# ec-jrc/lisflood-code

Hardware: AMD Instinct MI355X
Metric: Mcell-steps/s kinematic routing (higher is better)
Workload: dtype f64

## Files before the change

### lisflood-code_amd/csrc/lf_soil.hip

```cpp
#include <algorithm>
#include <cmath>
#include <cstdlib>

#include "lf_common.h"
#include "lf_canopy.h"
#include "lf_math.h"
#include "lf_soil_math.h"

namespace {

constexpr double kMaxSoilSubSteps = 1048576.0;

constexpr int kBlock = 256;
constexpr int kMaxVeg = 16;

__global__ void __launch_bounds__(kBlock) k_interception(lf_interception_args A)
{
    const long long pix = (long long)blockIdx.x * kBlock + threadIdx.x;
    if (pix >= A.N) return;
    const double rain = A.Rain[pix];
    for (long long veg = 0; veg < A.V; ++veg) {
        const long long i = veg * A.N + pix;
        const double lai = A.LAI[i];
        double smax;
        if (lai <= .1)
            smax = 0.;
        else if (lai <= 43.3)
            smax = 0.935 + 0.498 * lai - 0.00575 * (lai * lai);
        else
            smax = 11.718;
        double cum = A.CumInterception[i], inter;
        if (smax > 0) {
            double v = smax - cum;
            v = dmin(v, smax * (1. - exp(-0.046 * lai * rain / smax)));
            v = dmin(v, rain);
            inter = v;
            cum += inter;
        } else
            inter = 0.;
        double ta, drain;
        if (cum > 0.) {
            ta = dmax(dmin(cum, A.TaInterceptionMax[i]), 0.);
            cum = dmax(cum - ta, 0.);
            drain = A.drainageK * cum;
            cum = dmax(cum - drain, 0.);
        } else {
            ta = 0.;
            drain = 0.;
        }
        A.Interception[i] = inter;
        A.TaInterception[i] = ta;
        A.LeafDrainage[i] = drain;
        A.CumInterception[i] = cum;
    }
}

struct veg_plan {
    int mode[kMaxVeg];
    int landuse[kMaxVeg];
    int drained[kMaxVeg];
    int paddy_row[kMaxVeg];
};

constexpr int kClasses = 128;
constexpr int kLoopFields = 7 * 3 + 1;
constexpr int kColsPerWave = 20;
constexpr int kTile = 256;
#ifndef LF_STRAG_CAP
#define LF_STRAG_CAP 48
#endif
constexpr int kStragCap = LF_STRAG_CAP;
constexpr int kStragFields = 40;
#ifndef LF_STRAG_GROUP
#define LF_STRAG_GROUP 16
#endif
constexpr int kStragGroup = LF_STRAG_GROUP;

__device__ __forceinline__ double row_prev(double x)
{
    const int lo = __builtin_amdgcn_update_dpp(0, __double2loint(x), 0x111, 0xf, 0xf, true);
    const int hi = __builtin_amdgcn_update_dpp(0, __double2hiint(x), 0x111, 0xf, 0xf, true);
    return __hiloint2double(hi, lo);
}
__device__ __forceinline__ double row_next(double x)
{
    const int lo = __builtin_amdgcn_update_dpp(0, __double2loint(x), 0x101, 0xf, 0xf, true);
    const int hi = __builtin_amdgcn_update_dpp(0, __double2hiint(x), 0x101, 0xf, 0xf, true);
    return __hiloint2double(hi, lo);
}

template <bool FASTPOW>
__device__ __forceinline__ double layer_loop(unsigned int layer, double w, double wres, double ws, double ks, double im,
                                             double m, double k, bool pore, long long nsub, long long trips, double DtDay)
{
    const double dtsub = DtDay / (double)nsub;
    double av = w - wres, wt = w, cap = ws - w, sum = 0.;
#if LF_SOIL_HOISTED_RCP
    const soil_den D = soil_den_of(ws, wres);
#endif
    for (long long s = 0; s < trips; ++s) {
#if LF_SOIL_HOISTED_RCP
        if (s > 0) k = unsat_k_r<FASTPOW>(wt, pore, wres, D, ks, im, m);
#else
        if (s > 0) k = unsat_k<FASTPOW>(wt, pore, wres, ws, ks, im, m);
#endif
        const double cap_below = row_next(cap);
        const double limit = (layer == 2u) ? av : cap_below;
        const double flux = dmin(k * dtsub, limit);
        const double flux_above = row_prev(flux);
        const double net = (layer == 0u) ? -flux : flux_above - flux;
        const bool live = s < nsub;
        av = live ? av + net : av;
        wt = av + wres;
        cap = ws - wt;
        sum = live ? sum + flux : sum;
    }
    return sum;
}

struct soil_tail {
    double w1a, w1b, w2, inf, pref, uz, uzout, gwp, ws1a;
    double sd1a, sd1b, sd2, wwp1a, wwp1b, wwp1, wwp2, wfc1a, wfc1b, wfc1, wfc2;
    int flags;
};

__device__ __forceinline__ void soil_finish(const lf_soil_args &A, long long i, bool drained, const soil_tail &T, double sa,
                                            double sb, double sg)
{
    const bool frozen = (T.flags & 1) != 0, pore1a = (T.flags & 2) != 0, pore1b = (T.flags & 4) != 0, pore2 = (T.flags & 8) != 0;
    if (frozen) sa = sb = sg = 0.;
    double w1a = T.w1a - sa;
    const double w1b = T.w1b + sa - sb;
    const double w2 = T.w2 + sb - sg;
    const double w1 = w1a + w1b;
    const double inf = T.inf - dmax(w1a - T.ws1a, 0.);
    w1a = dmin(w1a, T.ws1a);
    double uz = T.uz, uzout = T.uzout;
    if (drained) {
        uzout += A.DrainedFraction * sg;
        uz += (1 - A.DrainedFraction) * sg + T.pref;
    } else
        uz += sg + T.pref;
    const double perc = dmin(T.gwp, uz);
    uz = dmax(uz - perc, 0.);
    A.SeepTopToSubA[i] = sa;
    A.SeepTopToSubB[i] = sb;
    A.SeepSubToGW[i] = sg;
    A.Infiltration[i] = inf;
    A.W1a[i] = w1a;
    A.W1b[i] = w1b;
    A.W1[i] = w1;
    A.W2[i] = w2;
    if (A.Theta1a) A.Theta1a[i] = pore1a ? w1a / T.sd1a : 0.;
    if (A.Theta1b) A.Theta1b[i] = pore1b ? w1b / T.sd1b : 0.;
    if (A.Theta2) A.Theta2[i] = pore2 ? w2 / T.sd2 : 0.;
    if (A.Sat1a) A.Sat1a[i] = (w1a - T.wwp1a) / (T.wfc1a - T.wwp1a);
    if (A.Sat1b) A.Sat1b[i] = (w1b - T.wwp1b) / (T.wfc1b - T.wwp1b);
    if (A.Sat1) A.Sat1[i] = (w1 - T.wwp1) / (T.wfc1 - T.wwp1);
    if (A.Sat2) A.Sat2[i] = (w2 - T.wwp2) / (T.wfc2 - T.wwp2);
    A.UZOutflow[i] = uzout;
    A.GwPercUZLZ[i] = perc;
    A.UZ[i] = uz;
}

struct soil_strag {
    double *rec;
    unsigned short *key;
    unsigned int *count;
    int trip_cap;
};

template <bool FASTPOW, bool DERIVED, bool CANOPY>
__global__ void __launch_bounds__(kTile) __attribute__((amdgpu_waves_per_eu(3)))
k_soil_fused(lf_soil_args A, veg_plan P, unsigned short *__restrict__ all_list, unsigned int *__restrict__ all_count,
             soil_strag G, unsigned int tile0, unsigned int tiles_per_veg, lf_canopy_args C, const double *__restrict__ ESRef)
{
    constexpr int kLoopCap = kTile / 2;
    __shared__ unsigned int s_count, s_next, s_all, s_strag;
    __shared__ double s_rec[kLoopFields * kLoopCap];
    __shared__ double s_res[3 * kLoopCap];
    __shared__ unsigned int s_key[kLoopCap];
    __shared__ unsigned short s_order[kLoopCap];
    __shared__ double s_stage[kStragFields * kStragCap];
    if (threadIdx.x == 0) {
        s_count = 0;
        s_next = 0;
        s_all = 0;
        s_strag = 0;
    }
    __syncthreads();
    const long long N = A.N;
    const double DtDay = A.DtDay;
    const unsigned int tile = tile0 + blockIdx.x;
    const int veg = (int)(tile / tiles_per_veg);
    const long long pix = (long long)(tile - (unsigned int)veg * tiles_per_veg) * kTile + threadIdx.x;
    const int mode = P.mode[veg];
    bool active = pix < N && mode != 0;
    if (active && mode == 2 && !A.paddy_inactive[(long long)P.paddy_row[veg] * N + pix]) active = false;
    const long long i = (long long)veg * N + pix, j = (long long)P.landuse[veg] * N + pix;

    soil_tail T;
    T.w1a = T.w1b = T.w2 = T.inf = T.pref = T.uz = T.uzout = T.gwp = T.ws1a = 0.;
    T.sd1a = T.sd1b = T.sd2 = 1.;
    T.wwp1a = T.wwp1b = T.wwp1 = T.wwp2 = 0.;
    T.wfc1a = T.wfc1b = T.wfc1 = T.wfc2 = 1.;
    T.flags = 0;
    double sa = 0, sb = 0, sg = 0;
    double k1a = 0, k1b = 0, k2 = 0, nsub_f = 1;
    unsigned int rank = 0xffffffffu;
    if (active) {
        const double in_rain = A.Rain[pix], in_snow = A.SnowMelt[pix];
        double in_leaf, in_int, in_w1a, in_w1b, in_w1, in_esmax;
        lf_canopy::column_in cin = {};
        double c_ewref = 0., c_etref = 0., c_esref = 0.;
        unsigned char c_frozen = 0;
        if (CANOPY) {
            cin = lf_canopy::load(C, veg, i, j);
            c_ewref = C.EWRef[pix];
            c_etref = C.ETRef[pix];
            c_esref = ESRef[pix];
            c_frozen = A.isFrozenSoil[pix];
        } else {
            in_leaf = A.LeafDrainage[i]; in_int = A.Interception[i];
            in_w1a = A.W1a[i]; in_w1b = A.W1b[i]; in_w1 = A.W1[i];
            in_esmax = A.ESMax[i];
        }
        const double in_dslr = A.DSLR[i], in_w2 = A.W2[i];
        const double in_uz = A.UZ[i];
        const double in_store = A.StoreMaxPervious[j];
        const double in_bx = A.b_Xinanjiang[pix], in_pinf = A.PowerInfPot[pix], in_ppref = A.PowerPrefFlow[pix];
        const double in_uzk = A.UpperZoneK[pix];
        T.gwp = A.GwPercStep[pix];
        T.sd1a = A.SoilDepth1a[j]; T.sd1b = A.SoilDepth1b[j]; T.sd2 = A.SoilDepth2[j];
        T.wwp1a = A.WWP1a[j]; T.wwp1b = A.WWP1b[j]; T.wwp2 = A.WWP2[j];
        T.wfc1a = A.WFC1a[j]; T.wfc1b = A.WFC1b[j]; T.wfc2 = A.WFC2[j];
        const double ks1a = A.KSat1a[j], ks1b = A.KSat1b[j], ks2 = A.KSat2[j];
        const double m1a = A.GenuM1a[j], m1b = A.GenuM1b[j], m2 = A.GenuM2[j];
        const double wres1a = A.WRes1a[j], wres1b = A.WRes1b[j], wres2 = A.WRes2[j];
        const double ws1a = A.WS1a[j], ws1b = A.WS1b[j], ws2 = A.WS2[j];
        T.ws1a = ws1a;
        if (CANOPY) {
            const lf_canopy::column_out o = lf_canopy::compute(C, veg, pix, i, j, cin, in_rain, c_ewref, c_etref, c_frozen != 0);
            in_leaf = o.leaf_drainage; in_int = o.interception;
            in_w1a = o.w1a; in_w1b = o.w1b; in_w1 = o.w1;
            in_esmax = c_esref * cin.lai_term;
        }
        const bool is_frozen = A.isFrozenSoil[pix] != 0;
        double im1a, im1b, im2, in_wres1, in_ws1;
        int flags;
        if (DERIVED) {
            im1a = 1 / m1a; im1b = 1 / m1b; im2 = 1 / m2;
            in_ws1 = ws1a + ws1b; in_wres1 = wres1a + wres1b;
            T.wfc1 = T.wfc1a + T.wfc1b; T.wwp1 = T.wwp1a + T.wwp1b;
            flags = (is_frozen ? 1 : 0) | ((T.sd1a != 0 && ws1a != 0) ? 2 : 0) | ((T.sd1b != 0 && ws1b != 0) ? 4 : 0) |
                    ((T.sd2 != 0 && ws2 != 0) ? 8 : 0);
        } else {
            im1a = A.GenuInvM1a[j]; im1b = A.GenuInvM1b[j]; im2 = A.GenuInvM2[j];
            in_ws1 = A.WS1[j]; in_wres1 = A.WRes1[j];
            T.wfc1 = A.WFC1[j]; T.wwp1 = A.WWP1[j];
            flags = (is_frozen ? 1 : 0) | (A.PoreSpaceNotZero1a[j] != 0 ? 2 : 0) | (A.PoreSpaceNotZero1b[j] != 0 ? 4 : 0) |
                    (A.PoreSpaceNotZero2[j] != 0 ? 8 : 0);
        }
        T.flags = flags;
        const bool frozen = (flags & 1) != 0, pore1a = (flags & 2) != 0, pore1b = (flags & 4) != 0, pore2 = (flags & 8) != 0;
        double awi = dmax((in_rain + in_snow) + in_leaf - in_int, 0.);
        double dslr = in_dslr;
        if (awi > A.AvWaterThreshold)
            dslr = 1;
        else
            dslr += DtDay;
        double esact, w1a = in_w1a, w1b = in_w1b;
        if (frozen)
            esact = 0.;
        else {
            esact = in_esmax * (sqrt(dslr) - sqrt(dslr - 1));
            esact = dmax(dmin(esact, in_w1 - in_wres1), 0.);
            const double supply1a = w1a - wres1a;
            const double es1a = dmin(esact, supply1a);
            const double es1b = dmax(esact - supply1a, 0.);
            w1a = dmax(w1a - es1a, wres1a);
            w1b = dmax(w1b - es1b, wres1b);
        }
        const double w1_ = w1a + w1b;
        const double relsat1 = pore1a ? dmin(w1_ / in_ws1, 1.0) : 0.0;
        const double satfrac = 1.0 - powxy<FASTPOW>(1.0 - relsat1, in_bx);
        const double infpot = frozen ? 0.0 : in_store * powxy<FASTPOW>(1. - satfrac, in_pinf) * DtDay;
        const double pref = powxy<FASTPOW>(relsat1, in_ppref) * awi;
        awi -= pref;
        const double inf = dmax(dmin(awi, infpot), 0.);
        const double test1a = w1a + inf;
        w1a = dmin(ws1a, test1a);
        w1b += dmax(test1a - ws1a, 0.);
        const double w2 = in_w2;
        T.w1a = w1a; T.w1b = w1b; T.w2 = w2; T.inf = inf; T.pref = pref;
        A.DSLR[i] = dslr;
        A.ESAct[i] = esact;
        A.PrefFlow[i] = pref;
        A.AvailableWaterForInfiltration[i] = awi;
        T.uzout = dmin(in_uzk * in_uz, in_uz);
        T.uz = dmax(in_uz - T.uzout, 0.);
        {
            const double w_[3] = {w1a, w1b, w2}, wres_[3] = {wres1a, wres1b, wres2}, ws_[3] = {ws1a, ws1b, ws2};
            const double ks_[3] = {ks1a, ks1b, ks2}, im_[3] = {im1a, im1b, im2}, m_[3] = {m1a, m1b, m2};
            const bool pore_[3] = {pore1a, pore1b, pore2};
            double k_[3];
            unsat_k3<FASTPOW>(w_, pore_, wres_, ws_, ks_, im_, m_, k_);
            k1a = k_[0], k1b = k_[1], k2 = k_[2];
        }
        const double av1a = w1a - wres1a, av1b = w1b - wres1b, av2 = w2 - wres2;
        const double ca = (av1a == 0) ? 0. : k1a * DtDay / av1a;
        const double cb = (av1b == 0) ? 0. : k1b * DtDay / av1b;
        const double cg = (av2 == 0) ? 0. : k2 * DtDay / av2;
        const double courant = dmax(dmax(ca, cb), cg);
        nsub_f = dmin(dmax(1., ceil(courant / A.CourantCrit)), kMaxSoilSubSteps);
#ifdef LF_SOIL_DEBUG_MAXTRIPS
        nsub_f = dmin(nsub_f, (double)LF_SOIL_DEBUG_MAXTRIPS);
#endif
        if (frozen) nsub_f = 1.;
        if (nsub_f > 1.) {
            long long c = (long long)nsub_f;
            c = c < kClasses - 1 ? c : kClasses - 1;
            const unsigned short key = (unsigned short)(threadIdx.x | ((int)c << 8));
            all_list[(size_t)tile * kTile + atomicAdd(&s_all, 1u)] = key;
            unsigned int sr = 0xffffffffu;
            if (G.trip_cap > 0 && nsub_f > (double)G.trip_cap) sr = atomicAdd(&s_strag, 1u);
            if (sr < (unsigned int)kStragCap) {
                double *R = s_stage + sr * kStragFields;
                R[0] = w1a; R[1] = wres1a; R[2] = ws1a; R[3] = ks1a; R[4] = im1a; R[5] = m1a; R[6] = k1a;
                R[7] = w1b; R[8] = wres1b; R[9] = ws1b; R[10] = ks1b; R[11] = im1b; R[12] = m1b; R[13] = k1b;
                R[14] = w2; R[15] = wres2; R[16] = ws2; R[17] = ks2; R[18] = im2; R[19] = m2; R[20] = k2;
                R[21] = (double)flags; R[22] = nsub_f; R[23] = (double)threadIdx.x;
                R[24] = inf; R[25] = pref; R[26] = T.uz; R[27] = T.uzout; R[28] = T.gwp;
                R[29] = T.sd1a; R[30] = T.sd1b; R[31] = T.sd2;
                R[32] = T.wwp1a; R[33] = T.wwp1b; R[34] = T.wwp1; R[35] = T.wwp2;
                R[36] = T.wfc1a; R[37] = T.wfc1b; R[38] = T.wfc1; R[39] = T.wfc2;
                G.key[(size_t)tile * kStragCap + sr] = key;
            } else {
                rank = atomicAdd(&s_count, 1u);
                if (rank < (unsigned int)kLoopCap) {
#define REC(f, v) s_rec[(f) * kLoopCap + rank] = (v)
                    REC(0, w1a); REC(1, wres1a); REC(2, ws1a); REC(3, ks1a); REC(4, im1a); REC(5, m1a); REC(6, k1a);
                    REC(7, w1b); REC(8, wres1b); REC(9, ws1b); REC(10, ks1b); REC(11, im1b); REC(12, m1b); REC(13, k1b);
                    REC(14, w2); REC(15, wres2); REC(16, ws2); REC(17, ks2); REC(18, im2); REC(19, m2); REC(20, k2);
                    REC(21, (double)flags);
#undef REC
                    s_key[rank] = (unsigned int)nsub_f;
                }
            }
        } else {
            sa = dmin(k1a * DtDay, ws1b - w1b);
            sb = dmin(k1b * DtDay, ws2 - w2);
            sg = dmin(k2 * DtDay, av2);
        }
    }
    __syncthreads();
    const unsigned int count = (unsigned int)__builtin_amdgcn_readfirstlane((int)s_count);
    {
        const unsigned int ns = s_strag < (unsigned int)kStragCap ? s_strag : (unsigned int)kStragCap;
        if (threadIdx.x == 0) {
            all_count[tile] = s_all;
            if (G.trip_cap > 0) G.count[tile] = ns;
        }
        double *dst = G.rec + (size_t)tile * kStragCap * kStragFields;
        for (unsigned int idx = threadIdx.x; idx < ns * kStragFields; idx += kTile) dst[idx] = s_stage[idx];
    }
    for (unsigned int base = 0; base < count; base += kLoopCap) {
        if (base > 0) {
            __syncthreads();
            if (threadIdx.x == 0) s_next = 0;
            const unsigned int r = rank - base;
            if (r < (unsigned int)kLoopCap) {
#define REC(f, v) s_rec[(f) * kLoopCap + r] = (v)
                REC(0, T.w1a); REC(1, A.WRes1a[j]); REC(2, T.ws1a); REC(3, A.KSat1a[j]); REC(4, DERIVED ? 1 / A.GenuM1a[j] : A.GenuInvM1a[j]); REC(5, A.GenuM1a[j]); REC(6, k1a);
                REC(7, T.w1b); REC(8, A.WRes1b[j]); REC(9, A.WS1b[j]); REC(10, A.KSat1b[j]); REC(11, DERIVED ? 1 / A.GenuM1b[j] : A.GenuInvM1b[j]); REC(12, A.GenuM1b[j]); REC(13, k1b);
                REC(14, T.w2); REC(15, A.WRes2[j]); REC(16, A.WS2[j]); REC(17, A.KSat2[j]); REC(18, DERIVED ? 1 / A.GenuM2[j] : A.GenuInvM2[j]); REC(19, A.GenuM2[j]); REC(20, k2);
                REC(21, (double)T.flags);
#undef REC
                s_key[r] = (unsigned int)nsub_f;
            }
            __syncthreads();
        }
        const unsigned int n = (count - base) < (unsigned int)kLoopCap ? (count - base) : (unsigned int)kLoopCap;
        if (threadIdx.x < n) {
            const unsigned int k = s_key[threadIdx.x];
            unsigned int pos = 0;
            for (unsigned int q = 0; q < n; ++q) {
                const unsigned int kq = s_key[q];
                pos += (kq > k || (kq == k && q < threadIdx.x)) ? 1u : 0u;
            }
            s_order[pos] = (unsigned short)threadIdx.x;
        }
        __syncthreads();
        const unsigned int ntasks = (n + kColsPerWave - 1) / kColsPerWave, lane = threadIdx.x & 63u;
        const unsigned int in_row = lane & 15u, col_in_row = in_row / 3u, layer = in_row - 3u * col_in_row;
        const unsigned int col = (lane >> 4) * 5u + col_in_row;
        for (;;) {
            unsigned int t = 0;
            if (lane == 0) t = atomicAdd(&s_next, 1u);
            t = (unsigned int)__builtin_amdgcn_readfirstlane((int)t);
            if (t >= ntasks) break;
            const unsigned int e = t * kColsPerWave + col;
            const bool valid = col_in_row < 5u && e < n;
            const unsigned int first = s_order[t * kColsPerWave];
            const unsigned int slot = valid ? s_order[e] : first;
            const double *__restrict__ R = s_rec + (7u * layer) * kLoopCap + slot;
            const double w = R[0], wres = R[kLoopCap], ws = R[2 * kLoopCap], ks = R[3 * kLoopCap], im = R[4 * kLoopCap],
                         m = R[5 * kLoopCap], k0 = R[6 * kLoopCap];
            const int fl = (int)s_rec[21 * kLoopCap + slot];
            const bool pore = ((fl >> (1 + (int)layer)) & 1) != 0;
            const long long trips = (long long)__builtin_amdgcn_readfirstlane((int)s_key[first]);
            const long long nsub = (long long)s_key[slot];
            const double sum = layer_loop<FASTPOW>(layer, w, wres, ws, ks, im, m, k0, pore, valid ? nsub : 0, trips, DtDay);
            if (valid) s_res[layer * kLoopCap + slot] = sum;
        }
        __syncthreads();
        const unsigned int r = rank - base;
        if (r < (unsigned int)kLoopCap) {
            sa = s_res[r];
            sb = s_res[kLoopCap + r];
            sg = s_res[2 * kLoopCap + r];
        }
    }
    if (!active) return;
    soil_finish(A, i, P.drained[veg] != 0, T, sa, sb, sg);
}

template <bool FASTPOW>
__global__ void __launch_bounds__(kTile) k_soil_stragglers(lf_soil_args A, veg_plan P, soil_strag G, unsigned int group0,
                                                           unsigned int ntiles, unsigned int tiles_per_veg)
{
    constexpr int kMaxEntries = kStragGroup * kStragCap;
    static_assert(kClasses <= kTile && kClasses % 64 == 0 && kStragCap < 256 && kStragGroup < 256, "list layout");
    __shared__ unsigned int off[kStragGroup + 1], h[kClasses], base[kClasses], next_task;
    __shared__ unsigned short cls_of[kMaxEntries], rank_of[kMaxEntries], ent_of[kMaxEntries];
    __shared__ unsigned short entry[kMaxEntries];
    const unsigned int t0 = (group0 + blockIdx.x) * kStragGroup;
    if (threadIdx.x < kClasses) h[threadIdx.x] = 0;
    if (threadIdx.x == 0) {
        unsigned int t = 0;
        for (int g = 0; g < kStragGroup; ++g) {
            off[g] = t;
            t += (t0 + g < ntiles) ? G.count[t0 + g] : 0;
        }
        off[kStragGroup] = t;
        next_task = 0;
    }
    __syncthreads();
    const unsigned int total = off[kStragGroup];
    if (total == 0) return;
    for (unsigned int q = threadIdx.x; q < total; q += kTile) {
        unsigned int g = 0;
        while (off[g + 1] <= q) ++g;
        const unsigned int sl = q - off[g];
        const unsigned int cls = G.key[(size_t)(t0 + g) * kStragCap + sl] >> 8;
        cls_of[q] = (unsigned short)cls;
        ent_of[q] = (unsigned short)((g << 8) | sl);
        rank_of[q] = (unsigned short)atomicAdd(&h[cls], 1u);
    }
    __syncthreads();
    if (threadIdx.x < 64) {
        constexpr int per = kClasses / 64;
        unsigned int mine_sum = 0;
#pragma unroll
        for (int q = 0; q < per; ++q) mine_sum += h[threadIdx.x * per + q];
        unsigned int incl = mine_sum;
#pragma unroll
        for (int d = 1; d < 64; d <<= 1) {
            const unsigned int up = __shfl_up(incl, d, 64);
            if ((int)threadIdx.x >= d) incl += up;
        }
        unsigned int acc = incl - mine_sum;
#pragma unroll
        for (int q = 0; q < per; ++q) {
            base[threadIdx.x * per + q] = acc;
            acc += h[threadIdx.x * per + q];
        }
    }
    __syncthreads();
    for (unsigned int q = threadIdx.x; q < total; q += kTile) entry[base[cls_of[q]] + rank_of[q]] = ent_of[q];
    __syncthreads();
    const unsigned int ntasks = (total + kColsPerWave - 1) / kColsPerWave, lane = threadIdx.x & 63u;
    const unsigned int in_row = lane & 15u, col_in_row = in_row / 3u, layer = in_row - 3u * col_in_row;
    const unsigned int col = (lane >> 4) * 5u + col_in_row;
    for (;;) {
        unsigned int t = 0;
        if (lane == 0) t = atomicAdd(&next_task, 1u);
        t = (unsigned int)__builtin_amdgcn_readfirstlane((int)t);
        if (t >= ntasks) break;
        const unsigned int e = t * kColsPerWave + col;
        const bool valid = col_in_row < 5u && e < total;
        const unsigned int ent = entry[total - 1u - (valid ? e : t * kColsPerWave)];
        const unsigned int tile = t0 + (ent >> 8);
        const double *__restrict__ R = G.rec + ((size_t)tile * kStragCap + (ent & 0xffu)) * kStragFields;
        const double *__restrict__ L = R + 7u * layer;
        const double w = L[0], wres = L[1], ws = L[2], ks = L[3], im = L[4], m = L[5], k0 = L[6];
        const int fl = (int)R[21];
        const bool pore = ((fl >> (1 + (int)layer)) & 1) != 0;
        const int nsub = valid ? (int)R[22] : 0;
        int trips = nsub;
#pragma unroll
        for (int d = 32; d >= 1; d >>= 1) {
            const int o = __shfl_xor(trips, d, 64);
            trips = o > trips ? o : trips;
        }
        const double sum = layer_loop<FASTPOW>(layer, w, wres, ws, ks, im, m, k0, pore, nsub, trips, A.DtDay);
        const double sb = row_next(sum);
        const double sg = row_next(sb);
        if (valid && layer == 0u) {
            soil_tail T;
            T.w1a = R[0]; T.w1b = R[7]; T.w2 = R[14]; T.ws1a = R[2]; T.flags = fl;
            T.inf = R[24]; T.pref = R[25]; T.uz = R[26]; T.uzout = R[27]; T.gwp = R[28];
            T.sd1a = R[29]; T.sd1b = R[30]; T.sd2 = R[31];
            T.wwp1a = R[32]; T.wwp1b = R[33]; T.wwp1 = R[34]; T.wwp2 = R[35];
            T.wfc1a = R[36]; T.wfc1b = R[37]; T.wfc1 = R[38]; T.wfc2 = R[39];
            const int veg = (int)(tile / tiles_per_veg);
            const long long pix = (long long)(tile - (unsigned int)veg * tiles_per_veg) * kTile + (long long)R[23];
            soil_finish(A, (long long)veg * A.N + pix, P.drained[veg] != 0, T, sum, sb, sg);
        }
    }
}

int make_plan(const lf_soil_args *a, const uint8_t *paddy_any, veg_plan *P)
{
    if (a->V > kMaxVeg) return lf_set_error(LF_E_INVALID, "V = %lld exceeds the supported maximum %d", (long long)a->V, kMaxVeg);
    int count_paddy = 0;
    for (int veg = 0; veg < (int)a->V; ++veg) {
        P->landuse[veg] = (int)a->index_landuse_all[veg];
        if (P->landuse[veg] < 0 || P->landuse[veg] >= a->L)
            return lf_set_error(LF_E_INVALID, "index_landuse_all[%d] = %d out of range", veg, P->landuse[veg]);
        P->paddy_row[veg] = 0;
        if (a->is_paddy_irrig && a->is_paddy_irrig[veg]) {
            if (!paddy_any || !paddy_any[count_paddy]) {
                P->mode[veg] = 0;
                P->drained[veg] = 0;
                continue;
            }
            P->mode[veg] = 2;
            P->drained[veg] = 0;
            P->paddy_row[veg] = count_paddy++;
        } else {
            P->mode[veg] = 1;
            P->drained[veg] = (a->is_irrigated && a->is_irrigated[veg] && a->DrainedFraction > 0) ? 1 : 0;
        }
    }
    return LF_OK;
}

inline int blocks_for(int64_t n) { return (int)((n + kBlock - 1) / kBlock); }
constexpr int kSoilTripCap = 6;

}

extern "C" {

int lf_interception_device(int device, const lf_interception_args *a)
{
    if (!a) return lf_set_error(LF_E_INVALID, "null argument");
    lf_device_ctx *c;
    LF_TRY(lf_ctx(device, &c));
    if (a->N > 0 && a->V > 0)
        hipLaunchKernelGGL(k_interception, dim3(blocks_for(a->N)), dim3(kBlock), 0, c->stream, *a);
    LF_HIP(hipGetLastError());
    return LF_OK;
}

struct soil_ws_layout {
    size_t all_count, all_list, s_count, s_key, s_rec, bytes;
};
static soil_ws_layout soil_layout(size_t ntiles)
{
    auto up = [](size_t x) { return (x + 255) & ~(size_t)255; };
    soil_ws_layout L;
    L.all_count = 0;
    L.all_list = up(sizeof(unsigned int) * (ntiles + 4));
    L.s_count = L.all_list + up(sizeof(unsigned short) * ntiles * kTile);
    L.s_key = L.s_count + up(sizeof(unsigned int) * (ntiles + 4));
    L.s_rec = L.s_key + up(sizeof(unsigned short) * ntiles * kStragCap);
    L.bytes = L.s_rec + sizeof(double) * ntiles * kStragCap * kStragFields;
    return L;
}

int lf_soil_last_deferred(int device, int64_t *count)
{
    if (!count) return lf_set_error(LF_E_INVALID, "null argument");
    lf_device_ctx *c;
    LF_TRY(lf_ctx(device, &c));
    *count = 0;
    if (!c->soil_ws || c->soil_ntiles == 0) return LF_OK;
    std::vector<unsigned int> h(c->soil_ntiles);
    LF_HIP(hipMemcpyAsync(h.data(), c->soil_ws, sizeof(unsigned int) * c->soil_ntiles, hipMemcpyDeviceToHost, c->stream));
    LF_HIP(hipStreamSynchronize(c->stream));
    int64_t tot = 0;
    for (unsigned int v : h) tot += v;
    *count = tot;
    return LF_OK;
}

int lf_soil_substep_histogram(int device, int64_t *hist, int nbins)
{
    if (!hist || nbins < 2) return lf_set_error(LF_E_INVALID, "null argument");
    lf_device_ctx *c;
    LF_TRY(lf_ctx(device, &c));
    for (int k = 0; k < nbins; ++k) hist[k] = 0;
    if (!c->soil_ws || c->soil_ntiles == 0) return LF_OK;
    const size_t nt = c->soil_ntiles;
    const soil_ws_layout L = soil_layout(nt);
    std::vector<unsigned int> cnt(nt);
    std::vector<unsigned short> lst(nt * kTile);
    LF_HIP(hipMemcpyAsync(cnt.data(), (const char *)c->soil_ws + L.all_count, sizeof(unsigned int) * nt, hipMemcpyDeviceToHost, c->stream));
    LF_HIP(hipMemcpyAsync(lst.data(), (const char *)c->soil_ws + L.all_list, sizeof(unsigned short) * nt * kTile,
                          hipMemcpyDeviceToHost, c->stream));
    LF_HIP(hipStreamSynchronize(c->stream));
    for (size_t t = 0; t < nt; ++t)
        for (unsigned int k = 0; k < cnt[t] && k < (unsigned int)kTile; ++k) {
            const int cls = lst[t * kTile + k] >> 8;
            hist[cls < nbins - 1 ? cls : nbins - 1] += 1;
        }
    return LF_OK;
}

static int soil_columns_device(int device, const lf_soil_args *a, bool derived, const lf_canopy_args *canopy = nullptr,
                               const double *esref = nullptr);

int lf_soil_columns_device(int device, const lf_soil_args *a) { return soil_columns_device(device, a, false); }

int lf_soil_columns_device_derived(int device, const lf_soil_args *a) { return soil_columns_device(device, a, true); }

int lf_land_columns_device(int device, const lf_canopy_args *canopy, const lf_soil_args *soil, const double *ESRef_dev, int derived)
{
    if (!canopy || !soil || !ESRef_dev || !canopy->index_landuse || !soil->index_landuse_all)
        return lf_set_error(LF_E_INVALID, "null argument");
    if (canopy->V != soil->V || canopy->N != soil->N || canopy->L != soil->L || soil->V != soil->L)
        return lf_set_error(LF_E_INVALID, "land columns: canopy and soil must have the same V = L and N");
    for (int v = 0; v < (int)soil->V; ++v)
        if (canopy->index_landuse[v] != v || soil->index_landuse_all[v] != v || (soil->is_paddy_irrig && soil->is_paddy_irrig[v]))
            return lf_set_error(LF_E_INVALID, "land columns: needs index_landuse[v] == v and no paddy fraction (use the "
                                "separate entry points otherwise)");
    if ((canopy->WFilla || canopy->WFillb) && (!canopy->WFilla || !canopy->WFillb || !canopy->WPF3a || !canopy->WPF3b))
        return lf_set_error(LF_E_INVALID, "wateruse: WFilla, WFillb, WPF3a and WPF3b are needed together");
    const bool same = canopy->W1a == soil->W1a && canopy->W1b == soil->W1b && canopy->W1 == soil->W1 &&
                      canopy->Interception == soil->Interception && canopy->LeafDrainage == soil->LeafDrainage &&
                      canopy->Rain == soil->Rain && canopy->isFrozenSoil == soil->isFrozenSoil &&
                      canopy->WWP1a == soil->WWP1a && canopy->WWP1b == soil->WWP1b && canopy->WFC1a == soil->WFC1a &&
                      canopy->WFC1b == soil->WFC1b;
    if (!same) return lf_set_error(LF_E_INVALID, "land columns: canopy and soil arguments name different vectors");
    return soil_columns_device(device, soil, derived != 0, canopy, ESRef_dev);
}

static int soil_columns_device(int device, const lf_soil_args *a, bool derived, const lf_canopy_args *canopy, const double *esref)
{
    if (!a || !a->index_landuse_all) return lf_set_error(LF_E_INVALID, "null argument");
    lf_device_ctx *c;
    LF_TRY(lf_ctx(device, &c));
    veg_plan P;
    LF_TRY(make_plan(a, a->paddy_any, &P));
    if (a->N <= 0 || a->V <= 0) return LF_OK;
    if (!(a->CourantCrit > 0.0) || !(a->DtDay > 0.0))
        return lf_set_error(LF_E_INVALID, "CourantCrit and DtDay must be positive (soilloop.py:249: NoSubS = "
                            "ceil(Courant / CourantCrit))");
    if ((unsigned long long)a->V * (unsigned long long)a->N >= 0xffffffffull)
        return lf_set_error(LF_E_INVALID, "V*N exceeds the 32-bit column id range");
    const unsigned int tiles_per_veg = (unsigned int)((a->N + kTile - 1) / kTile);
    const size_t ntiles = (size_t)tiles_per_veg * (size_t)a->V;
    const soil_ws_layout L = soil_layout(ntiles);
    if (c->soil_ws_bytes < L.bytes) {
        if (c->soil_ws) LF_HIP(hipFree(c->soil_ws));
        c->soil_ws = nullptr;
        c->soil_ws_bytes = 0;
        LF_HIP(hipMalloc(&c->soil_ws, L.bytes));
        c->soil_ws_bytes = L.bytes;
    }
    c->soil_ntiles = ntiles;
    char *ws = (char *)c->soil_ws;
    unsigned int *all_count = (unsigned int *)(ws + L.all_count);
    unsigned short *all_list = (unsigned short *)(ws + L.all_list);
    soil_strag G;
    G.count = (unsigned int *)(ws + L.s_count);
    G.key = (unsigned short *)(ws + L.s_key);
    G.rec = (double *)(ws + L.s_rec);
    G.trip_cap = kSoilTripCap;
    if (const char *e = std::getenv("LF_SOIL_TRIP_CAP")) G.trip_cap = (int)std::atol(e) > 0 ? (int)std::atol(e) : 0;
    const char *force_general = std::getenv("LF_GENERAL_POW");
    const bool fastpow = !(force_general && force_general[0] == '1');
    const dim3 grid((unsigned)ntiles), block(kTile);
    size_t dyn = 0;
    if (const char *e = std::getenv("LF_SOIL_DEBUG_LDS")) dyn = (size_t)std::atol(e);
    if (const char *e = std::getenv("LF_SOIL_NO_DERIVED")) derived = derived && e[0] != '1';
    lf_canopy_args C{};
    if (canopy) C = *canopy;
#define LF_SOIL_LAUNCH(FP, DR, CN)                                                                                        \
    hipLaunchKernelGGL((k_soil_fused<FP, DR, CN>), grid, block, dyn, c->stream, *a, P, all_list, all_count, G, 0u,       \
                       tiles_per_veg, C, esref)
    if (canopy) {
        if (fastpow && derived) LF_SOIL_LAUNCH(true, true, true);
        else if (fastpow) LF_SOIL_LAUNCH(true, false, true);
        else if (derived) LF_SOIL_LAUNCH(false, true, true);
        else LF_SOIL_LAUNCH(false, false, true);
    } else {
        if (fastpow && derived) LF_SOIL_LAUNCH(true, true, false);
        else if (fastpow) LF_SOIL_LAUNCH(true, false, false);
        else if (derived) LF_SOIL_LAUNCH(false, true, false);
        else LF_SOIL_LAUNCH(false, false, false);
    }
#undef LF_SOIL_LAUNCH
    if (G.trip_cap > 0) {
        const dim3 grid2((unsigned)((ntiles + kStragGroup - 1) / kStragGroup));
        if (fastpow)
            hipLaunchKernelGGL(k_soil_stragglers<true>, grid2, block, 0, c->stream, *a, P, G, 0u, (unsigned int)ntiles, tiles_per_veg);
        else
            hipLaunchKernelGGL(k_soil_stragglers<false>, grid2, block, 0, c->stream, *a, P, G, 0u, (unsigned int)ntiles, tiles_per_veg);
    }
    LF_HIP(hipGetLastError());
    return LF_OK;
}

}


namespace {
struct stager {
    hipStream_t s;
    std::vector<void *> bufs;
    struct wb {
        void *host;
        void *dev;
        size_t bytes;
    };
    std::vector<wb> writeback;
    lf_device_ctx *ctx = nullptr;
    size_t used = 0;
    ~stager()
    {
        for (void *p : bufs) (void)hipFree(p);
        if (ctx) ctx->stage_need = used > ctx->stage_need ? used : ctx->stage_need;
    }
    int begin(lf_device_ctx *c)
    {
        ctx = c;
        if (c->stage_need > c->stage_bytes) {
            LF_HIP(hipStreamSynchronize(s));
            if (c->stage_base) (void)hipFree(c->stage_base);
            c->stage_base = nullptr;
            c->stage_bytes = 0;
            const size_t want = c->stage_need + c->stage_need / 8;
            if (hipMalloc(&c->stage_base, want) == hipSuccess)
                c->stage_bytes = want;
            else
                (void)hipGetLastError();
        }
        return LF_OK;
    }
    int carve(size_t bytes, void **out)
    {
        const size_t need = (bytes + 8 + 255) & ~(size_t)255;
        if (ctx && used + need <= ctx->stage_bytes) {
            *out = (char *)ctx->stage_base + used;
            used += need;
            return LF_OK;
        }
        used += need;
        LF_HIP(hipMalloc(out, need));
        bufs.push_back(*out);
        return LF_OK;
    }
    template <typename T>
    int in(const T *&field, size_t count)
    {
        if (!field) return lf_set_error(LF_E_INVALID, "null array argument");
        void *d = nullptr;
        LF_TRY(carve(count * sizeof(T), &d));
        LF_HIP(hipMemcpyAsync(d, field, count * sizeof(T), hipMemcpyHostToDevice, s));
        field = (const T *)d;
        return LF_OK;
    }
    template <typename T>
    int inout(T *&field, size_t count)
    {
        if (!field) return lf_set_error(LF_E_INVALID, "null array argument");
        void *d = nullptr;
        LF_TRY(carve(count * sizeof(T), &d));
        LF_HIP(hipMemcpyAsync(d, field, count * sizeof(T), hipMemcpyHostToDevice, s));
        writeback.push_back({(void *)field, d, count * sizeof(T)});
        field = (T *)d;
        return LF_OK;
    }
    int finish()
    {
        for (const wb &w : writeback) LF_HIP(hipMemcpyAsync(w.host, w.dev, w.bytes, hipMemcpyDeviceToHost, s));
        LF_HIP(hipStreamSynchronize(s));
        return LF_OK;
    }
};
}

extern "C" {

int lf_interception_host(int device, const lf_interception_args *a_in)
{
    if (!a_in) return lf_set_error(LF_E_INVALID, "null argument");
    lf_device_ctx *c;
    LF_TRY(lf_ctx(device, &c));
    lf_interception_args a = *a_in;
    stager st{c->stream, {}, {}};
    LF_TRY(st.begin(c));
    const size_t vn = (size_t)(a.V * a.N), n = (size_t)a.N;
    LF_TRY(st.inout(a.Interception, vn));
    LF_TRY(st.inout(a.TaInterception, vn));
    LF_TRY(st.inout(a.LeafDrainage, vn));
    LF_TRY(st.inout(a.CumInterception, vn));
    LF_TRY(st.in(a.LAI, vn));
    LF_TRY(st.in(a.Rain, n));
    LF_TRY(st.in(a.TaInterceptionMax, vn));
    LF_TRY(lf_interception_device(device, &a));
    return st.finish();
}

int lf_soil_columns_host(int device, const lf_soil_args *a_in)
{
    if (!a_in || !a_in->index_landuse_all) return lf_set_error(LF_E_INVALID, "null argument");
    lf_device_ctx *c;
    LF_TRY(lf_ctx(device, &c));
    lf_soil_args a = *a_in;
    stager st{c->stream, {}, {}};
    LF_TRY(st.begin(c));
    const size_t vn = (size_t)(a.V * a.N), ln = (size_t)(a.L * a.N), n = (size_t)a.N;
    std::vector<uint8_t> any;
    int n_paddy = 0;
    if (a.is_paddy_irrig)
        for (int v = 0; v < (int)a.V; ++v) n_paddy += a.is_paddy_irrig[v] != 0;
    if (n_paddy > 0) {
        if (!a.paddy_inactive) return lf_set_error(LF_E_INVALID, "paddy_inactive is required when is_paddy_irrig is set");
        any.assign(n_paddy, 0);
        for (int r = 0; r < n_paddy; ++r)
            for (size_t p = 0; p < n && !any[r]; ++p) any[r] = a.paddy_inactive[(size_t)r * n + p] != 0;
        LF_TRY(st.in(a.paddy_inactive, (size_t)n_paddy * n));
        a.paddy_any = any.data();
    } else {
        a.paddy_inactive = nullptr;
        a.paddy_any = nullptr;
    }
#define LF_IN_L(f) LF_TRY(st.in(a.f, ln))
#define LF_IN_N(f) LF_TRY(st.in(a.f, n))
#define LF_IN_V(f) LF_TRY(st.in(a.f, vn))
#define LF_IO_V(f) LF_TRY(st.inout(a.f, vn))
    LF_IN_L(PoreSpaceNotZero1a); LF_IN_L(PoreSpaceNotZero1b); LF_IN_L(PoreSpaceNotZero2);
    LF_IN_L(KSat1a); LF_IN_L(KSat1b); LF_IN_L(KSat2);
    LF_IN_L(GenuInvM1a); LF_IN_L(GenuInvM1b); LF_IN_L(GenuInvM2);
    LF_IN_L(GenuM1a); LF_IN_L(GenuM1b); LF_IN_L(GenuM2);
    LF_IN_L(WRes1a); LF_IN_L(WRes1b); LF_IN_L(WRes1); LF_IN_L(WRes2);
    LF_IN_L(WWP1a); LF_IN_L(WWP1b); LF_IN_L(WWP1); LF_IN_L(WWP2);
    LF_IN_L(WFC1a); LF_IN_L(WFC1b); LF_IN_L(WFC1); LF_IN_L(WFC2);
    LF_IN_L(SoilDepth1a); LF_IN_L(SoilDepth1b); LF_IN_L(SoilDepth2);
    LF_IN_L(WS1a); LF_IN_L(WS1b); LF_IN_L(WS1); LF_IN_L(WS2); LF_IN_L(StoreMaxPervious);
    LF_IN_N(Rain); LF_IN_N(SnowMelt); LF_IN_N(b_Xinanjiang); LF_IN_N(PowerInfPot); LF_IN_N(PowerPrefFlow);
    LF_IN_N(UpperZoneK); LF_IN_N(GwPercStep); LF_IN_N(isFrozenSoil);
    LF_IN_V(LeafDrainage); LF_IN_V(Interception); LF_IN_V(ESMax);
    LF_IO_V(AvailableWaterForInfiltration); LF_IO_V(DSLR); LF_IO_V(ESAct); LF_IO_V(PrefFlow); LF_IO_V(Infiltration);
    LF_IO_V(W1a); LF_IO_V(W1b); LF_IO_V(W1); LF_IO_V(W2);
    LF_IO_V(Theta1a); LF_IO_V(Theta1b); LF_IO_V(Theta2);
    LF_IO_V(Sat1a); LF_IO_V(Sat1b); LF_IO_V(Sat1); LF_IO_V(Sat2);
    LF_IO_V(SeepTopToSubA); LF_IO_V(SeepTopToSubB); LF_IO_V(SeepSubToGW);
    LF_IO_V(UZOutflow); LF_IO_V(UZ); LF_IO_V(GwPercUZLZ);
#undef LF_IN_L
#undef LF_IN_N
#undef LF_IN_V
#undef LF_IO_V
    LF_TRY(lf_soil_columns_device(device, &a));
    return st.finish();
}

}
```

Before: 107,800.

## Cut soil kernel register pressure by parking statics in LDS and reloading late

Reduces live state in the fused soil kernel so it can run at more waves per EU. Static soil parameters are parked in shared memory and UZ, percolation and WFC/WWP values are loaded only at finish time. Column indices are recomputed behind asm barriers, and flags are packed into the sub-step key. Straggler records are written straight to global memory instead of being staged, and overflow k values are kept in shared memory rather than registers. The cost is extra LDS traffic and repeated global loads, and the metric named (kinematic routing) may not exercise this soil kernel at all.

Result: no change. 107,900 (median of 3 runs) (+0.1%).

```diff
diff --git a/lisflood-code_amd/csrc/lf_soil.hip b/lisflood-code_amd/csrc/lf_soil.hip
--- a/lisflood-code_amd/csrc/lf_soil.hip
+++ b/lisflood-code_amd/csrc/lf_soil.hip
@@ -63,7 +63,8 @@
 };
 
 constexpr int kClasses = 128;
-constexpr int kLoopFields = 7 * 3 + 1;
+constexpr int kLoopFields = 7 * 3;
+constexpr unsigned int kFlagShift = 24, kTripMask = (1u << kFlagShift) - 1u;
 constexpr int kColsPerWave = 20;
 constexpr int kTile = 256;
 #ifndef LF_STRAG_CAP
@@ -74,6 +75,10 @@
 #ifndef LF_STRAG_GROUP
 #define LF_STRAG_GROUP 16
 #endif
+#ifndef LF_SOIL_WAVES
+#define LF_SOIL_WAVES 4
+#endif
+constexpr int kParkFields = 7;
 constexpr int kStragGroup = LF_STRAG_GROUP;
 
 __device__ __forceinline__ double row_prev(double x)
@@ -118,11 +123,33 @@
     return sum;
 }
 
+struct soil_statics {
+    double sd1a, sd1b, sd2, wwp1a, wwp1b, wwp1, wwp2, wfc1a, wfc1b, wfc1, wfc2;
+};
 struct soil_tail {
     double w1a, w1b, w2, inf, pref, uz, uzout, gwp, ws1a;
-    double sd1a, sd1b, sd2, wwp1a, wwp1b, wwp1, wwp2, wfc1a, wfc1b, wfc1, wfc2;
+    soil_statics S;
     int flags;
 };
+
+template <bool DERIVED>
+__device__ __forceinline__ void soil_tail_late(const lf_soil_args &A, long long i, long long j, long long pix,
+                                               const double *park, soil_tail &T)
+{
+    const double in_uz = A.UZ[i], in_uzk = A.UpperZoneK[pix];
+    T.gwp = A.GwPercStep[pix];
+    soil_statics &S = T.S;
+    S.sd1a = park[0]; S.sd1b = park[kTile]; S.sd2 = park[2 * kTile];
+    S.wwp1a = park[3 * kTile]; S.wwp1b = park[4 * kTile]; S.wfc1a = park[5 * kTile]; S.wfc1b = park[6 * kTile];
+    S.wwp2 = A.Sat2 ? A.WWP2[j] : 0.; S.wfc2 = A.Sat2 ? A.WFC2[j] : 1.;
+    if (DERIVED) {
+        S.wfc1 = S.wfc1a + S.wfc1b; S.wwp1 = S.wwp1a + S.wwp1b;
+    } else {
+        S.wfc1 = A.Sat1 ? A.WFC1[j] : 1.; S.wwp1 = A.Sat1 ? A.WWP1[j] : 0.;
+    }
+    T.uzout = dmin(in_uzk * in_uz, in_uz);
+    T.uz = dmax(in_uz - T.uzout, 0.);
+}
 
 __device__ __forceinline__ void soil_finish(const lf_soil_args &A, long long i, bool drained, const soil_tail &T, double sa,
                                             double sb, double sg)
@@ -151,13 +178,13 @@
     A.W1b[i] = w1b;
     A.W1[i] = w1;
     A.W2[i] = w2;
-    if (A.Theta1a) A.Theta1a[i] = pore1a ? w1a / T.sd1a : 0.;
-    if (A.Theta1b) A.Theta1b[i] = pore1b ? w1b / T.sd1b : 0.;
-    if (A.Theta2) A.Theta2[i] = pore2 ? w2 / T.sd2 : 0.;
-    if (A.Sat1a) A.Sat1a[i] = (w1a - T.wwp1a) / (T.wfc1a - T.wwp1a);
-    if (A.Sat1b) A.Sat1b[i] = (w1b - T.wwp1b) / (T.wfc1b - T.wwp1b);
-    if (A.Sat1) A.Sat1[i] = (w1 - T.wwp1) / (T.wfc1 - T.wwp1);
-    if (A.Sat2) A.Sat2[i] = (w2 - T.wwp2) / (T.wfc2 - T.wwp2);
+    if (A.Theta1a) A.Theta1a[i] = pore1a ? w1a / T.S.sd1a : 0.;
+    if (A.Theta1b) A.Theta1b[i] = pore1b ? w1b / T.S.sd1b : 0.;
+    if (A.Theta2) A.Theta2[i] = pore2 ? w2 / T.S.sd2 : 0.;
+    if (A.Sat1a) A.Sat1a[i] = (w1a - T.S.wwp1a) / (T.S.wfc1a - T.S.wwp1a);
+    if (A.Sat1b) A.Sat1b[i] = (w1b - T.S.wwp1b) / (T.S.wfc1b - T.S.wwp1b);
+    if (A.Sat1) A.Sat1[i] = (w1 - T.S.wwp1) / (T.S.wfc1 - T.S.wwp1);
+    if (A.Sat2) A.Sat2[i] = (w2 - T.S.wwp2) / (T.S.wfc2 - T.S.wwp2);
     A.UZOutflow[i] = uzout;
     A.GwPercUZLZ[i] = perc;
     A.UZ[i] = uz;
@@ -170,18 +197,34 @@
     int trip_cap;
 };
 
+struct soil_idx {
+    long long pix, i, j;
+};
+template <int PLACE>
+__device__ __forceinline__ soil_idx soil_idx_again(unsigned int tile_in_veg, int veg, int landuse, long long N)
+{
+    unsigned int t = threadIdx.x;
+    asm("; column indices again, place %1" : "+v"(t) : "i"(PLACE));
+    soil_idx X;
+    X.pix = (long long)tile_in_veg * kTile + t;
+    X.i = (long long)veg * N + X.pix;
+    X.j = (long long)landuse * N + X.pix;
+    return X;
+}
+
 template <bool FASTPOW, bool DERIVED, bool CANOPY>
-__global__ void __launch_bounds__(kTile) __attribute__((amdgpu_waves_per_eu(3)))
+__global__ void __launch_bounds__(kTile) __attribute__((amdgpu_waves_per_eu(LF_SOIL_WAVES)))
 k_soil_fused(lf_soil_args A, veg_plan P, unsigned short *__restrict__ all_list, unsigned int *__restrict__ all_count,
              soil_strag G, unsigned int tile0, unsigned int tiles_per_veg, lf_canopy_args C, const double *__restrict__ ESRef)
 {
     constexpr int kLoopCap = kTile / 2;
     __shared__ unsigned int s_count, s_next, s_all, s_strag;
     __shared__ double s_rec[kLoopFields * kLoopCap];
-    __shared__ double s_res[3 * kLoopCap];
     __shared__ unsigned int s_key[kLoopCap];
+    __shared__ double s_late_k[3 * kLoopCap];
+    __shared__ unsigned int s_late_key[kLoopCap];
     __shared__ unsigned short s_order[kLoopCap];
-    __shared__ double s_stage[kStragFields * kStragCap];
+    __shared__ double s_park[kParkFields * kTile];
     if (threadIdx.x == 0) {
         s_count = 0;
         s_next = 0;
@@ -189,6 +232,8 @@
         s_strag = 0;
     }
     __syncthreads();
+#define PARK(f, v) s_park[(f) * kTile + threadIdx.x] = (v)
+#define PARKED(f) s_park[(f) * kTile + threadIdx.x]
     const long long N = A.N;
     const double DtDay = A.DtDay;
     const unsigned int tile = tile0 + blockIdx.x;
@@ -197,13 +242,12 @@
     const int mode = P.mode[veg];
     bool active = pix < N && mode != 0;
     if (active && mode == 2 && !A.paddy_inactive[(long long)P.paddy_row[veg] * N + pix]) active = false;
-    const long long i = (long long)veg * N + pix, j = (long long)P.landuse[veg] * N + pix;
+    const int landuse = P.landuse[veg];
+    const unsigned int tile_in_veg = tile - (unsigned int)veg * tiles_per_veg;
+    const long long i = (long long)veg * N + pix, j = (long long)landuse * N + pix;
 
     soil_tail T;
     T.w1a = T.w1b = T.w2 = T.inf = T.pref = T.uz = T.uzout = T.gwp = T.ws1a = 0.;
-    T.sd1a = T.sd1b = T.sd2 = 1.;
-    T.wwp1a = T.wwp1b = T.wwp1 = T.wwp2 = 0.;
-    T.wfc1a = T.wfc1b = T.wfc1 = T.wfc2 = 1.;
     T.flags = 0;
     double sa = 0, sb = 0, sg = 0;
     double k1a = 0, k1b = 0, k2 = 0, nsub_f = 1;
@@ -226,40 +270,39 @@
             in_esmax = A.ESMax[i];
         }
         const double in_dslr = A.DSLR[i], in_w2 = A.W2[i];
-        const double in_uz = A.UZ[i];
         const double in_store = A.StoreMaxPervious[j];
         const double in_bx = A.b_Xinanjiang[pix], in_pinf = A.PowerInfPot[pix], in_ppref = A.PowerPrefFlow[pix];
-        const double in_uzk = A.UpperZoneK[pix];
-        T.gwp = A.GwPercStep[pix];
-        T.sd1a = A.SoilDepth1a[j]; T.sd1b = A.SoilDepth1b[j]; T.sd2 = A.SoilDepth2[j];
-        T.wwp1a = A.WWP1a[j]; T.wwp1b = A.WWP1b[j]; T.wwp2 = A.WWP2[j];
-        T.wfc1a = A.WFC1a[j]; T.wfc1b = A.WFC1b[j]; T.wfc2 = A.WFC2[j];
+        const double sd1a = A.SoilDepth1a[j], sd1b = A.SoilDepth1b[j], sd2 = A.SoilDepth2[j];
+        const double wwp1a = A.WWP1a[j], wwp1b = A.WWP1b[j], wfc1a = A.WFC1a[j], wfc1b = A.WFC1b[j];
         const double ks1a = A.KSat1a[j], ks1b = A.KSat1b[j], ks2 = A.KSat2[j];
         const double m1a = A.GenuM1a[j], m1b = A.GenuM1b[j], m2 = A.GenuM2[j];
         const double wres1a = A.WRes1a[j], wres1b = A.WRes1b[j], wres2 = A.WRes2[j];
         const double ws1a = A.WS1a[j], ws1b = A.WS1b[j], ws2 = A.WS2[j];
         T.ws1a = ws1a;
+        __builtin_amdgcn_sched_barrier(0);
+        PARK(0, sd1a); PARK(1, sd1b); PARK(2, sd2);
+        PARK(3, wwp1a); PARK(4, wwp1b); PARK(5, wfc1a); PARK(6, wfc1b);
         if (CANOPY) {
-            const lf_canopy::column_out o = lf_canopy::compute(C, veg, pix, i, j, cin, in_rain, c_ewref, c_etref, c_frozen != 0);
+            const soil_idx Xc = soil_idx_again<1>(tile_in_veg, veg, landuse, N);
+            const lf_canopy::column_out o = lf_canopy::compute(C, veg, Xc.pix, Xc.i, Xc.j, cin, in_rain, c_ewref, c_etref, c_frozen != 0);
             in_leaf = o.leaf_drainage; in_int = o.interception;
             in_w1a = o.w1a; in_w1b = o.w1b; in_w1 = o.w1;
             in_esmax = c_esref * cin.lai_term;
         }
-        const bool is_frozen = A.isFrozenSoil[pix] != 0;
+        const soil_idx X = soil_idx_again<2>(tile_in_veg, veg, landuse, N);
+        const bool is_frozen = A.isFrozenSoil[X.pix] != 0;
         double im1a, im1b, im2, in_wres1, in_ws1;
         int flags;
         if (DERIVED) {
             im1a = 1 / m1a; im1b = 1 / m1b; im2 = 1 / m2;
             in_ws1 = ws1a + ws1b; in_wres1 = wres1a + wres1b;
-            T.wfc1 = T.wfc1a + T.wfc1b; T.wwp1 = T.wwp1a + T.wwp1b;
-            flags = (is_frozen ? 1 : 0) | ((T.sd1a != 0 && ws1a != 0) ? 2 : 0) | ((T.sd1b != 0 && ws1b != 0) ? 4 : 0) |
-                    ((T.sd2 != 0 && ws2 != 0) ? 8 : 0);
+            flags = (is_frozen ? 1 : 0) | ((sd1a != 0 && ws1a != 0) ? 2 : 0) | ((sd1b != 0 && ws1b != 0) ? 4 : 0) |
+                    ((sd2 != 0 && ws2 != 0) ? 8 : 0);
         } else {
-            im1a = A.GenuInvM1a[j]; im1b = A.GenuInvM1b[j]; im2 = A.GenuInvM2[j];
-            in_ws1 = A.WS1[j]; in_wres1 = A.WRes1[j];
-            T.wfc1 = A.WFC1[j]; T.wwp1 = A.WWP1[j];
-            flags = (is_frozen ? 1 : 0) | (A.PoreSpaceNotZero1a[j] != 0 ? 2 : 0) | (A.PoreSpaceNotZero1b[j] != 0 ? 4 : 0) |
-                    (A.PoreSpaceNotZero2[j] != 0 ? 8 : 0);
+            im1a = A.GenuInvM1a[X.j]; im1b = A.GenuInvM1b[X.j]; im2 = A.GenuInvM2[X.j];
+            in_ws1 = A.WS1[X.j]; in_wres1 = A.WRes1[X.j];
+            flags = (is_frozen ? 1 : 0) | (A.PoreSpaceNotZero1a[X.j] != 0 ? 2 : 0) | (A.PoreSpaceNotZero1b[X.j] != 0 ? 4 : 0) |
+                    (A.PoreSpaceNotZero2[X.j] != 0 ? 8 : 0);
         }
         T.flags = flags;
         const bool frozen = (flags & 1) != 0, pore1a = (flags & 2) != 0, pore1b = (flags & 4) != 0, pore2 = (flags & 8) != 0;
@@ -293,12 +336,10 @@
         w1b += dmax(test1a - ws1a, 0.);
         const double w2 = in_w2;
         T.w1a = w1a; T.w1b = w1b; T.w2 = w2; T.inf = inf; T.pref = pref;
-        A.DSLR[i] = dslr;
-        A.ESAct[i] = esact;
-        A.PrefFlow[i] = pref;
-        A.AvailableWaterForInfiltration[i] = awi;
-        T.uzout = dmin(in_uzk * in_uz, in_uz);
-        T.uz = dmax(in_uz - T.uzout, 0.);
+        A.DSLR[X.i] = dslr;
+        A.ESAct[X.i] = esact;
+        A.PrefFlow[X.i] = pref;
+        A.AvailableWaterForInfiltration[X.i] = awi;
         {
             const double w_[3] = {w1a, w1b, w2}, wres_[3] = {wres1a, wres1b, wres2}, ws_[3] = {ws1a, ws1b, ws2};
             const double ks_[3] = {ks1a, ks1b, ks2}, im_[3] = {im1a, im1b, im2}, m_[3] = {m1a, m1b, m2};
@@ -325,15 +366,17 @@
             unsigned int sr = 0xffffffffu;
             if (G.trip_cap > 0 && nsub_f > (double)G.trip_cap) sr = atomicAdd(&s_strag, 1u);
             if (sr < (unsigned int)kStragCap) {
-                double *R = s_stage + sr * kStragFields;
+                double *R = G.rec + ((size_t)tile * kStragCap + sr) * kStragFields;
                 R[0] = w1a; R[1] = wres1a; R[2] = ws1a; R[3] = ks1a; R[4] = im1a; R[5] = m1a; R[6] = k1a;
                 R[7] = w1b; R[8] = wres1b; R[9] = ws1b; R[10] = ks1b; R[11] = im1b; R[12] = m1b; R[13] = k1b;
                 R[14] = w2; R[15] = wres2; R[16] = ws2; R[17] = ks2; R[18] = im2; R[19] = m2; R[20] = k2;
                 R[21] = (double)flags; R[22] = nsub_f; R[23] = (double)threadIdx.x;
                 R[24] = inf; R[25] = pref; R[26] = T.uz; R[27] = T.uzout; R[28] = T.gwp;
-                R[29] = T.sd1a; R[30] = T.sd1b; R[31] = T.sd2;
-                R[32] = T.wwp1a; R[33] = T.wwp1b; R[34] = T.wwp1; R[35] = T.wwp2;
-                R[36] = T.wfc1a; R[37] = T.wfc1b; R[38] = T.wfc1; R[39] = T.wfc2;
+                soil_tail_late<DERIVED>(A, X.i, X.j, X.pix, s_park + threadIdx.x, T);
+                const soil_statics &S = T.S;
+                R[29] = S.sd1a; R[30] = S.sd1b; R[31] = S.sd2;
+                R[32] = S.wwp1a; R[33] = S.wwp1b; R[34] = S.wwp1; R[35] = S.wwp2;
+                R[36] = S.wfc1a; R[37] = S.wfc1b; R[38] = S.wfc1; R[39] = S.wfc2;
                 G.key[(size_t)tile * kStragCap + sr] = key;
             } else {
                 rank = atomicAdd(&s_count, 1u);
@@ -342,9 +385,12 @@
                     REC(0, w1a); REC(1, wres1a); REC(2, ws1a); REC(3, ks1a); REC(4, im1a); REC(5, m1a); REC(6, k1a);
                     REC(7, w1b); REC(8, wres1b); REC(9, ws1b); REC(10, ks1b); REC(11, im1b); REC(12, m1b); REC(13, k1b);
                     REC(14, w2); REC(15, wres2); REC(16, ws2); REC(17, ks2); REC(18, im2); REC(19, m2); REC(20, k2);
-                    REC(21, (double)flags);
 #undef REC
-                    s_key[rank] = (unsigned int)nsub_f;
+                    s_key[rank] = (unsigned int)nsub_f | ((unsigned int)flags << kFlagShift);
+                } else {
+                    const unsigned int r = rank - (unsigned int)kLoopCap;
+                    s_late_k[r] = k1a; s_late_k[kLoopCap + r] = k1b; s_late_k[2 * kLoopCap + r] = k2;
+                    s_late_key[r] = (unsigned int)nsub_f | ((unsigned int)flags << kFlagShift);
                 }
             }
         } else {
@@ -361,31 +407,29 @@
             all_count[tile] = s_all;
             if (G.trip_cap > 0) G.count[tile] = ns;
         }
-        double *dst = G.rec + (size_t)tile * kStragCap * kStragFields;
-        for (unsigned int idx = threadIdx.x; idx < ns * kStragFields; idx += kTile) dst[idx] = s_stage[idx];
     }
     for (unsigned int base = 0; base < count; base += kLoopCap) {
         if (base > 0) {
             __syncthreads();
             if (threadIdx.x == 0) s_next = 0;
             const unsigned int r = rank - base;
+            const soil_idx X = soil_idx_again<3>(tile_in_veg, veg, landuse, N);
             if (r < (unsigned int)kLoopCap) {
 #define REC(f, v) s_rec[(f) * kLoopCap + r] = (v)
-                REC(0, T.w1a); REC(1, A.WRes1a[j]); REC(2, T.ws1a); REC(3, A.KSat1a[j]); REC(4, DERIVED ? 1 / A.GenuM1a[j] : A.GenuInvM1a[j]); REC(5, A.GenuM1a[j]); REC(6, k1a);
-                REC(7, T.w1b); REC(8, A.WRes1b[j]); REC(9, A.WS1b[j]); REC(10, A.KSat1b[j]); REC(11, DERIVED ? 1 / A.GenuM1b[j] : A.GenuInvM1b[j]); REC(12, A.GenuM1b[j]); REC(13, k1b);
-                REC(14, T.w2); REC(15, A.WRes2[j]); REC(16, A.WS2[j]); REC(17, A.KSat2[j]); REC(18, DERIVED ? 1 / A.GenuM2[j] : A.GenuInvM2[j]); REC(19, A.GenuM2[j]); REC(20, k2);
-                REC(21, (double)T.flags);
+                REC(0, T.w1a); REC(1, A.WRes1a[X.j]); REC(2, T.ws1a); REC(3, A.KSat1a[X.j]); REC(4, DERIVED ? 1 / A.GenuM1a[X.j] : A.GenuInvM1a[X.j]); REC(5, A.GenuM1a[X.j]); REC(6, s_late_k[r]);
+                REC(7, T.w1b); REC(8, A.WRes1b[X.j]); REC(9, A.WS1b[X.j]); REC(10, A.KSat1b[X.j]); REC(11, DERIVED ? 1 / A.GenuM1b[X.j] : A.GenuInvM1b[X.j]); REC(12, A.GenuM1b[X.j]); REC(13, s_late_k[kLoopCap + r]);
+                REC(14, T.w2); REC(15, A.WRes2[X.j]); REC(16, A.WS2[X.j]); REC(17, A.KSat2[X.j]); REC(18, DERIVED ? 1 / A.GenuM2[X.j] : A.GenuInvM2[X.j]); REC(19, A.GenuM2[X.j]); REC(20, s_late_k[2 * kLoopCap + r]);
 #undef REC
-                s_key[r] = (unsigned int)nsub_f;
+                s_key[r] = s_late_key[r];
             }
             __syncthreads();
         }
         const unsigned int n = (count - base) < (unsigned int)kLoopCap ? (count - base) : (unsigned int)kLoopCap;
         if (threadIdx.x < n) {
-            const unsigned int k = s_key[threadIdx.x];
+            const unsigned int k = s_key[threadIdx.x] & kTripMask;
             unsigned int pos = 0;
             for (unsigned int q = 0; q < n; ++q) {
-                const unsigned int kq = s_key[q];
+                const unsigned int kq = s_key[q] & kTripMask;
                 pos += (kq > k || (kq == k && q < threadIdx.x)) ? 1u : 0u;
             }
             s_order[pos] = (unsigned short)threadIdx.x;
@@ -406,23 +450,27 @@
             const double *__restrict__ R = s_rec + (7u * layer) * kLoopCap + slot;
             const double w = R[0], wres = R[kLoopCap], ws = R[2 * kLoopCap], ks = R[3 * kLoopCap], im = R[4 * kLoopCap],
                          m = R[5 * kLoopCap], k0 = R[6 * kLoopCap];
-            const int fl = (int)s_rec[21 * kLoopCap + slot];
-            const bool pore = ((fl >> (1 + (int)layer)) & 1) != 0;
-            const long long trips = (long long)__builtin_amdgcn_readfirstlane((int)s_key[first]);
-            const long long nsub = (long long)s_key[slot];
+            const unsigned int key = s_key[slot];
+            const bool pore = ((key >> (kFlagShift + 1u + layer)) & 1u) != 0;
+            const long long trips = (long long)__builtin_amdgcn_readfirstlane((int)(s_key[first] & kTripMask));
+            const long long nsub = (long long)(key & kTripMask);
             const double sum = layer_loop<FASTPOW>(layer, w, wres, ws, ks, im, m, k0, pore, valid ? nsub : 0, trips, DtDay);
-            if (valid) s_res[layer * kLoopCap + slot] = sum;
+            if (valid) s_rec[(7u * layer) * kLoopCap + slot] = sum;
         }
         __syncthreads();
         const unsigned int r = rank - base;
         if (r < (unsigned int)kLoopCap) {
-            sa = s_res[r];
-            sb = s_res[kLoopCap + r];
-            sg = s_res[2 * kLoopCap + r];
+            sa = s_rec[r];
+            sb = s_rec[7 * kLoopCap + r];
+            sg = s_rec[14 * kLoopCap + r];
         }
     }
     if (!active) return;
-    soil_finish(A, i, P.drained[veg] != 0, T, sa, sb, sg);
+    const soil_idx X = soil_idx_again<4>(tile_in_veg, veg, landuse, N);
+    soil_tail_late<DERIVED>(A, X.i, X.j, X.pix, s_park + threadIdx.x, T);
+#undef PARK
+#undef PARKED
+    soil_finish(A, X.i, P.drained[veg] != 0, T, sa, sb, sg);
 }
 
 template <bool FASTPOW>
@@ -510,9 +558,9 @@
             soil_tail T;
             T.w1a = R[0]; T.w1b = R[7]; T.w2 = R[14]; T.ws1a = R[2]; T.flags = fl;
             T.inf = R[24]; T.pref = R[25]; T.uz = R[26]; T.uzout = R[27]; T.gwp = R[28];
-            T.sd1a = R[29]; T.sd1b = R[30]; T.sd2 = R[31];
-            T.wwp1a = R[32]; T.wwp1b = R[33]; T.wwp1 = R[34]; T.wwp2 = R[35];
-            T.wfc1a = R[36]; T.wfc1b = R[37]; T.wfc1 = R[38]; T.wfc2 = R[39];
+            T.S.sd1a = R[29]; T.S.sd1b = R[30]; T.S.sd2 = R[31];
+            T.S.wwp1a = R[32]; T.S.wwp1b = R[33]; T.S.wwp1 = R[34]; T.S.wwp2 = R[35];
+            T.S.wfc1a = R[36]; T.S.wfc1b = R[37]; T.S.wfc1 = R[38]; T.S.wfc2 = R[39];
             const int veg = (int)(tile / tiles_per_veg);
             const long long pix = (long long)(tile - (unsigned int)veg * tiles_per_veg) * kTile + (long long)R[23];
             soil_finish(A, (long long)veg * A.N + pix, P.drained[veg] != 0, T, sum, sb, sg);
```
